# akanazawa/human_dynamics

Measured on AMD Instinct MI355X. Metric: frames/sec/GPU (ResNet+temporal+SMPL, 224x224); SMPL verts max-abs-err, higher is better.
Workload: dtype f16x3

## Files before the change

human_dynamics_amd/_lib.py:

```python
from __future__ import annotations

import ctypes as C
import os

from . import devflags

HERE = os.path.dirname(os.path.abspath(__file__))
LIB_PATH = devflags.get("LIB_PATH") or os.path.join(HERE, "libhmmr_hip.so")

HMMR_F32, HMMR_BF16, HMMR_F16X3 = 0, 1, 2
FLAG_SATURATED = 1
FLAG_NAN = 2
ABI_VERSION = 19
RESNET_UNITS = 16
RESNET_PROF_SLOTS = 64
MAX_TEMPORAL_BLOCKS = 8
MAX_REGRESSORS = 8

_vp, _fp, _ip = C.c_void_p, C.c_void_p, C.c_void_p


class ConvDesc(C.Structure):
    _fields_ = [
        ("in_", _vp), ("w", _vp), ("scale", _fp), ("shift", _fp), ("res", _vp), ("out", _vp),
        ("out2", _vp), ("scale2", _fp), ("shift2", _fp),
        ("in_dtype", C.c_int), ("out_dtype", C.c_int),
        ("n_img", C.c_int), ("hin", C.c_int), ("win", C.c_int), ("cin", C.c_int),
        ("in_img_stride", C.c_int64), ("in_row_stride", C.c_int), ("in_px_stride", C.c_int),
        ("kh", C.c_int), ("kw", C.c_int), ("sy", C.c_int), ("sx", C.c_int), ("py", C.c_int), ("px", C.c_int),
        ("ho", C.c_int), ("wo", C.c_int), ("cout", C.c_int), ("ldo", C.c_int),
        ("ldr", C.c_int), ("res_strided", C.c_int), ("res_img_stride", C.c_int64),
        ("res_row_stride", C.c_int), ("res_px_stride", C.c_int),
        ("relu", C.c_int), ("tile", C.c_int),
        ("split_k", C.c_int), ("ws", _vp), ("ws_bytes", C.c_size_t),
        ("pro_scale", _fp), ("pro_shift", _fp),
        ("out_b", _vp), ("ldo_b", C.c_int), ("n_split", C.c_int), ("relu_b", C.c_int),
        ("in2", _vp), ("cin2", C.c_int), ("k_order", C.c_int),
        ("batch", C.c_int), ("batch_in_bytes", C.c_int64), ("batch_w_bytes", C.c_int64), ("batch_out_bytes", C.c_int64),
        ("batch_res_bytes", C.c_int64), ("batch_scale_bytes", C.c_int64), ("batch_shift_bytes", C.c_int64),
    ]


class TailDesc(C.Structure):
    _fields_ = [
        ("dtype", C.c_int), ("h2", _vp), ("m", C.c_int), ("c_mid", C.c_int), ("depth", C.c_int),
        ("w3", _vp), ("scale3", _fp), ("shift3", _fp),
        ("res", _vp), ("ldr", C.c_int), ("res_strided", C.c_int), ("res_img_stride", C.c_int64),
        ("res_row_stride", C.c_int), ("res_px_stride", C.c_int), ("ho", C.c_int), ("wo", C.c_int),
        ("out", _vp), ("pre_scale", _fp), ("pre_shift", _fp),
        ("w1", _vp), ("scale1", _fp), ("shift1", _fp), ("relu1", C.c_int), ("n2", C.c_int),
        ("out_h1", _vp),
        ("h1", _vp), ("hin", C.c_int), ("win", C.c_int), ("w2", _vp), ("scale2", _fp), ("shift2", _fp),
        ("xp", _vp), ("wsc", _vp), ("shift_sc", _fp),
        ("conv2_stride", C.c_int), ("out_pre", _vp),
        ("pair_stream", _vp), ("c_xp", C.c_int), ("unit_stream", _vp), ("trunk_keep_stride", C.c_int),
    ]


class Debug(C.Structure):
    _fields_ = [("stem_route", C.c_int), ("stem_no_conv1", C.c_int), ("gemm_probe", C.c_int), ("smpl_blend_mfma", C.c_int), ("ief_no_group", C.c_int), ("reserved", C.c_int * 2), ("keep_dead_rows", C.c_int),
                ("pair_min_pixels", C.c_int), ("pair_two_tile_min", C.c_int), ("pair_form", C.c_int)]


class LaunchCounts(C.Structure):
    _fields_ = [("unit_pair", C.c_ulonglong), ("b1_unit", C.c_ulonglong), ("tail_split", C.c_ulonglong), ("conv3x3_stream", C.c_ulonglong),
                ("conv1x1_stream", C.c_ulonglong)]


class StemCounts(C.Structure):
    _fields_ = [(k, C.c_ulonglong) for k in ("fused", "fused_conv1", "repack", "gemm", "pool")]


TILE_GENERIC, TILE_PATCH, TILE_STREAM_3X3, TILE_STREAM_1X1 = range(4)
CONV_TILE_MAX = 63


class ConvTileInfo(C.Structure):
    _fields_ = [(k, C.c_int) for k in ("tile", "family", "fm", "fn", "wgm", "wgn", "pixels", "channels", "row_blocks", "depth", "occupancy", "wmax",
                                       "split_only", "conv3_form", "cols", "tune_cols", "narrow", "rank", "candidate")] + [("text", C.c_char_p)]


class Layer(C.Structure):
    _fields_ = [("w", _vp), ("scale", _fp), ("shift", _fp), ("tile", C.c_int), ("k_order", C.c_int)]


class ResnetUnit(C.Structure):
    _fields_ = [("conv1", Layer), ("conv2", Layer), ("conv3", Layer), ("shortcut", Layer), ("c3sc", Layer), ("sc_c1", Layer),
                ("w3_frag", _vp), ("w1n_frag", _vp), ("pair_stream", _vp), ("conv1_frag", _vp), ("unit_stream", _vp), ("pre_scale", _fp), ("pre_shift", _fp),
                ("c_in", C.c_int), ("base", C.c_int), ("depth", C.c_int), ("stride", C.c_int),
                ("fuse_preact", C.c_int), ("fuse_tail", C.c_int)]


class ResnetWeights(C.Structure):
    _fields_ = [("dtype", C.c_int), ("stem", Layer),
                ("unit", ResnetUnit * RESNET_UNITS), ("post_scale", _fp), ("post_shift", _fp)]


SC_NONE, SC_LAUNCH, SC_LAUNCH_WITH_CONV1, SC_IN_CONV3, SC_IN_TAIL = range(5)
CONV1_LAUNCH, CONV1_READY = range(2)
CONV2_LAUNCH, CONV2_IN_TAIL = range(2)
END_CONV3_LAUNCH, END_TAIL_BF16, END_TAIL_BF16_STRIDE2, END_TAIL_SPLIT, END_B1_UNIT, END_UNIT_PAIR = range(6)


class UnitPlan(C.Structure):
    _fields_ = [(k, C.c_int) for k in ("shortcut", "conv1", "conv2", "end", "reads_fused_preact", "writes_raw", "writes_pre",
                                       "pair_demoted", "swaps_t1_t2", "leaves_h1", "trunk_keep_stride")]


def resnet_plan(rw, n_total):
    plan = (UnitPlan * RESNET_UNITS)()
    check(load().hmmr_resnet50_plan(C.byref(rw), int(n_total), plan), "hmmr_resnet50_plan")
    return list(plan)

# ... 366 lines not shown
```

human_dynamics_amd/build.py:

```python
from __future__ import annotations

import os
import subprocess
import sys
from concurrent.futures import ThreadPoolExecutor

HERE = os.path.dirname(os.path.abspath(__file__))
CSRC = os.path.join(HERE, "csrc")
INCLUDE = os.path.join(os.path.dirname(HERE), "include")
LIB = os.path.join(HERE, "libhmmr_hip.so")
SOURCES = ["api.cpp", "pack.cpp", "gemm_conv.hip", "conv3x3_stream.hip", "conv1x1_stream.hip", "stem.hip", "bottleneck.hip", "bottleneck_split.hip", "unit_pair.hip", "b1_unit.hip", "resnet.hip", "temporal.hip", "ief.hip", "ief_grad.hip", "movie_grad.hip", "disc_pose.hip", "smpl.hip", "smpl_grad.hip", "losses.hip", "adam.hip", "eval_metrics.hip", "preprocess.hip", "tube.hip", "track.hip", "handoff.hip", "render.hip", "collage.hip", "person_view.hip", "windows.hip", "video_plan.cpp", "video.cpp", "probe.hip"]
HIPCC = os.environ.get("HIPCC", "/opt/rocm/bin/hipcc")
FLAGS = ["--offload-arch=gfx950", "-O3", "-std=c++17", "-fPIC", "-fno-slp-vectorize", "-I", INCLUDE, "-I", CSRC,
         "-Wall", "-Wno-unused-function"]


EXTRA_FLAGS = {"pack.cpp": ["-ffp-contract=off"], "track.hip": ["-ffp-contract=off"], "collage.hip": ["-ffp-contract=off"],
               "tube.hip": ["-ffp-contract=off"], "person_view.hip": ["-ffp-contract=off"], "adam.hip": ["-ffp-contract=off"]}


def _newer(src, dst):
    return (not os.path.exists(dst)) or os.path.getmtime(src) > os.path.getmtime(dst)


def _deps():
    return sorted(os.path.join(d, h) for d in (CSRC, INCLUDE) for h in os.listdir(d) if h.endswith(".h"))


def build(force=False, verbose=True):
    objs, jobs = [], []
    for src in SOURCES:
        s = os.path.join(CSRC, src)
        o = os.path.join(CSRC, os.path.splitext(src)[0] + ".o")
        objs.append(o)
        if force or _newer(s, o) or any(_newer(d, o) for d in _deps()):
            lang = ["-x", "hip"] if src.endswith(".hip") else []
            jobs.append([HIPCC] + FLAGS + EXTRA_FLAGS.get(src, []) + lang + ["-c", s, "-o", o])

    def run(cmd):
        if verbose:
            print(" ".join(cmd), flush=True)
        r = subprocess.run(cmd, stdout=subprocess.PIPE, stderr=subprocess.STDOUT, text=True)
        if r.returncode != 0:
            raise RuntimeError("hipcc failed:\n%s\n%s" % (" ".join(cmd), r.stdout))
        if verbose and r.stdout.strip():
            print(r.stdout)

    if jobs:
        with ThreadPoolExecutor(max_workers=min(len(jobs), os.cpu_count() or 4)) as ex:
            list(ex.map(run, jobs))
    if jobs or force or not os.path.exists(LIB):
        run([HIPCC, "--offload-arch=gfx950", "-shared", "-fPIC", "-o", LIB] + objs)
        from . import isa_check
        unsafe = isa_check.unsafe_forms(LIB)
        if unsafe:
            os.replace(LIB, LIB + ".rejected")
            raise RuntimeError("the linked library holds packed-fp32 instructions gfx950 gets wrong beside MFMAs (isa_check.py, DESIGN 4.6); "
                               "kept as %s.rejected:\n%s" % (LIB, "\n".join("  %d x %s %s in %s" % (n, op, mods, kern)
                                                                             for (kern, op, mods), n in sorted(unsafe.items()))))
        if verbose:
            print("isa_check: %s" % ("no disassembler (%s) or no gfx950 code object found in the library: NOT checked" % isa_check.OBJDUMP if unsafe is None
                                     else "no packed-fp32 instruction reads source 1's high register into its low result"), flush=True)
    return LIB

# ... 4 lines not shown
```

human_dynamics_amd/csrc/gemm_conv.hip:

```cpp
#include <stdlib.h>
#include <string.h>
#include <type_traits>

#include "conv_tiles.h"
#include "stream_kit.h"

struct ConvArgs {
    const void* in; const void* w; const float* scale; const float* shift;
    const void* res; void* out; void* out2; const float* scale2; const float* shift2;
    const float* pro_scale; const float* pro_shift;
    void* out_b; int ldo_b, n_split, relu_b;
    int M, K, cout, ldo, ldr;
    int Wo, HoWo, Hin, Win;
    long long in_img_stride; int in_row_stride, in_px_stride;
    int cin_log2, KH, KW, SY, SX, PY, PX;
    int res_strided; long long res_img_stride; int res_row_stride, res_px_stride;
    int relu, tiles_n, n_tiles;
    int kt_per_slice;
    long long out_slice_stride;
    int probe;
    const void* in2; int cin2, kt_split;
    int batch; long long bz_in, bz_w, bz_out, bz_res, bz_scale, bz_shift;
};

__device__ __forceinline__ ConvArgs batch_problem(const ConvArgs& a0, int z) {
    ConvArgs a = a0;
    if (a0.batch > 1) {
        const long long zz = z;
        a.in = (const char*)a0.in + zz * a0.bz_in;
        a.w = (const char*)a0.w + zz * a0.bz_w;
        if (a0.out) a.out = (char*)a0.out + zz * a0.bz_out;
        if (a0.out2) a.out2 = (char*)a0.out2 + zz * a0.bz_out;
        if (a0.res) a.res = (const char*)a0.res + zz * a0.bz_res;
        if (a0.scale) a.scale = (const float*)((const char*)a0.scale + zz * a0.bz_scale);
        if (a0.shift) a.shift = (const float*)((const char*)a0.shift + zz * a0.bz_shift);
        if (a0.scale2) a.scale2 = (const float*)((const char*)a0.scale2 + zz * a0.bz_scale);
        if (a0.shift2) a.shift2 = (const float*)((const char*)a0.shift2 + zz * a0.bz_shift);
    }
    return a;
}

#ifdef HMMR_GEMM_PROBE
#define HMMR_PROBE(a, bit) (((a).probe & (bit)) != 0)
#else
#define HMMR_PROBE(a, bit) false
#endif

template <typename TA> struct Frag;
template <> struct Frag<float>  { typedef f32x4 type; };
template <> struct Frag<bf16_t> { typedef bf16x8 type; };
struct split_frag { shalf8 hi, lo; };
template <> struct Frag<bsplit_t> { typedef split_frag type; };

__device__ __forceinline__ f32x16 mma(const f32x4& a, const f32x4& b, f32x16 c) {
#pragma unroll
    for (int j = 0; j < 4; ++j) c = __builtin_amdgcn_mfma_f32_32x32x2f32(a[j], b[j], c, 0, 0, 0);
    return c;
}
__device__ __forceinline__ f32x16 mma(const bf16x8& a, const bf16x8& b, f32x16 c) {
    return __builtin_amdgcn_mfma_f32_32x32x16_bf16(a, b, c, 0, 0, 0);
}
__device__ __forceinline__ f32x16 mma(const split_frag& a, const split_frag& b, f32x16 c) {
    c = mfma_split(a.lo, b.hi, c);
    c = mfma_split(a.hi, b.lo, c);
    return mfma_split(a.hi, b.hi, c);
}
template <typename TA> struct FragIO {
    static constexpr int CHUNKS = 4;
    __device__ static __forceinline__ typename Frag<TA>::type read(const char* row, int c, int lh, int fsw) {
        return *(const typename Frag<TA>::type*)(row + (((2 * c + lh) ^ fsw) << 4));
    }
};
template <> struct FragIO<bsplit_t> {
    static constexpr int CHUNKS = 2;
    __device__ static __forceinline__ split_frag read(const char* row, int c, int lh, int fsw) {
        const int g = 2 * (2 * c + lh);
        split_frag f;
        f.hi = *(const shalf8*)(row + ((g ^ fsw) << 4));
        f.lo = *(const shalf8*)(row + (((g + 1) ^ fsw) << 4));
        return f;
    }
};
template <typename TO> __device__ __forceinline__ void store_tail(TO* p, const float (&v)[8], int cnt) {
    if constexpr (!std::is_same<TO, bsplit_t>::value)
        for (int j = 0; j < cnt; ++j) p[j] = elem_traits<TO>::from_f32(v[j]);
}

__device__ const u32x4 g_zero_page[4] = {};

template <typename TA> __device__ __forceinline__ u32x4 preact_slot(const u32x4& v, const f32x4* sc, const f32x4* sh);
template <> __device__ __forceinline__ u32x4 preact_slot<float>(const u32x4& v, const f32x4* sc, const f32x4* sh) {
    u32x4 o;
#pragma unroll
    for (int i = 0; i < 4; ++i) o[i] = __float_as_uint(fmaxf(fmaf(__uint_as_float(v[i]), sc[0][i], sh[0][i]), 0.f));
    return o;
}
template <> __device__ __forceinline__ u32x4 preact_slot<bf16_t>(const u32x4& v, const f32x4* sc, const f32x4* sh) {
    u32x4 o;
#pragma unroll
    for (int i = 0; i < 4; ++i) {
        const float lo = __uint_as_float(v[i] << 16), hi = __uint_as_float(v[i] & 0xffff0000u);
        const int e = 2 * i;
        const float a = fmaxf(fmaf(lo, sc[e >> 2][e & 3], sh[e >> 2][e & 3]), 0.f);
        const float b = fmaxf(fmaf(hi, sc[(e + 1) >> 2][(e + 1) & 3], sh[(e + 1) >> 2][(e + 1) & 3]), 0.f);
        typedef __attribute__((ext_vector_type(2))) __bf16 bf16x2;
        bf16x2 pk = {(bf16_t)a, (bf16_t)b};
        o[i] = __builtin_bit_cast(unsigned, pk);
    }
    return o;
}


template <typename TA, typename TO, int BM, int BN, int WGM, int WGN, bool PRO, bool UTAP, int NSTAGE>
__global__ __launch_bounds__(WGM * WGN * 64, NSTAGE >= 3 ? (WGM * WGN) / 4 : ((WGM * WGN == 8) ? 4 : 1))
void conv_gemm_kernel(const ConvArgs a0) {
    const ConvArgs a = batch_problem(a0, blockIdx.z);
    static_assert(NSTAGE >= 2 && NSTAGE <= 4, "2 stages (two workgroups per CU) or a 3/4-stage ring (one workgroup per CU)");
    static_assert(NSTAGE == 2 || WGM * WGN == 8, "the deep ring is written for 8-wave workgroups");
    static_assert(!PRO || UTAP, "the fused pre-activation needs one tap per K step");
// ... 1030 lines not shown
```

human_dynamics_amd/csrc/ief.hip:

```cpp
#include "common.h"
#include "hmmr_hip.h"
#include "tail_sched.h"
#include "workspace.h"

template <typename TO>
__global__ void cast_rows_kernel(const float* __restrict__ in, TO* __restrict__ out, long long n8) {
    const long long i = (long long)blockIdx.x * blockDim.x + threadIdx.x;
    if (i >= n8) return;
    float v[8];
    load8(in + i * 8, v);
    store8(out + i * 8, v);
}

__global__ void ief_init_theta_kernel(const float* __restrict__ src, int ld_src, int off, int nd,
                                      float* __restrict__ theta, float* __restrict__ theta_other, int m, long long th_stride) {
    const long long i = (long long)blockIdx.x * blockDim.x + threadIdx.x;
    if (i >= (long long)m * LDT) return;
    const int row = (int)(i / LDT), col = (int)(i % LDT);
    const long long z = (long long)blockIdx.y * th_stride;
    theta[z + i] = col < nd ? src[(long long)row * ld_src + off + col] : 0.f;
    theta_other[z + i] = 0.f;
}

__global__ void ief_finalize_kernel(const float* __restrict__ theta, const float* __restrict__ bsrc, int ld_b,
// ... 44 lines not shown
extern "C" int hmmr_ief_fwd_from(const hmmr_ief_weights_t* w, const float* strips, const float* omega_start, int m,
                                 float* omegas, void* ws, size_t ws_bytes, void* stream) {
    HMMR_REQUIRE(w && strips && omegas && ws, "hmmr_ief_fwd: null argument");
    HMMR_REQUIRE(m > 0, "hmmr_ief_fwd: m must be positive");
    HMMR_REQUIRE(w->num_regressors >= 1 && w->num_regressors <= HMMR_MAX_REGRESSORS, "hmmr_ief_fwd: bad num_regressors");
    HMMR_REQUIRE(w->reg[0].nd == 85, "hmmr_ief_fwd: regressor 0 must predict 85-D omega");
    const int nd_delta = w->no_optcam ? 75 : 72;
    for (int r = 0; r < w->num_regressors; ++r)
        HMMR_REQUIRE(w->reg[r].nd == (r == 0 ? 85 : nd_delta), "hmmr_ief_fwd: regressor %d has nd=%d (expected %d)", r,
                     w->reg[r].nd, r == 0 ? 85 : nd_delta);
    const IefBufs L = ief_layout(m, w->dtype, w->num_regressors - 1);
    HMMR_REQUIRE(ws_bytes >= L.total, "hmmr_ief_fwd: workspace too small");
    hipStream_t s = (hipStream_t)stream;
    char* base = (char*)ws;
    const void* xin = strips;
    if (w->dtype != HMMR_F32) {
        const long long n8 = (long long)m * 2048 / 8;
        if (w->dtype == HMMR_BF16)
            hipLaunchKernelGGL(cast_rows_kernel<bf16_t>, dim3((unsigned)((n8 + 255) / 256)), dim3(256), 0, s, strips,
                               (bf16_t*)(base + L.xin), n8);
        else
            hipLaunchKernelGGL(cast_rows_kernel<bsplit_t>, dim3((unsigned)((n8 + 255) / 256)), dim3(256), 0, s, strips,
                               (bsplit_t*)(base + L.xin), n8);
        HMMR_CHECK_HIP(hipGetLastError());
        xin = base + L.xin;
    }
    void* pre = base + L.pre; void* h1 = base + L.h1; void* h2 = base + L.h2;
    float* th[2] = {(float*)(base + L.th[0]), (float*)(base + L.th[1])};
    const unsigned gth = (unsigned)(((long long)m * LDT + 255) / 256);
    const unsigned gfin = (unsigned)(((long long)m * 85 + 255) / 256);
    const int nd_group = w->num_regressors - 1;
    struct Strides { long long w, scale, shift; };
    auto strides_of = [&](const hmmr_layer_t hmmr_ief_regressor_t::*lay, Strides& st) -> bool {
        st = Strides{0, 0, 0};
        for (int r = 2; r < w->num_regressors; ++r) {
            const hmmr_layer_t& a = w->reg[r - 1].*lay; const hmmr_layer_t& b = w->reg[r].*lay;
            const Strides cur = {(const char*)b.w - (const char*)a.w,
                                 a.scale ? (const char*)b.scale - (const char*)a.scale : 0,
                                 a.shift ? (const char*)b.shift - (const char*)a.shift : 0};
            if (!a.scale != !b.scale || !a.shift != !b.shift) return false;
            if (r > 2 && (cur.w != st.w || cur.scale != st.scale || cur.shift != st.shift)) return false;
            st = cur;
        }
        return ((st.w | st.scale | st.shift) & 15) == 0;
    };
    Strides s_phi, s_th, s_fc2, s_fc3;
    const bool grouped = nd_group >= 2 && !hmmr_debug_state()->ief_no_group &&
                         strides_of(&hmmr_ief_regressor_t::fc1_phi, s_phi) && strides_of(&hmmr_ief_regressor_t::fc1_theta, s_th) &&
                         strides_of(&hmmr_ief_regressor_t::fc2, s_fc2) && strides_of(&hmmr_ief_regressor_t::fc3, s_fc3);
    const float* start = omega_start ? omega_start : w->mean_theta;
    const int ld_start = omega_start ? 85 : 0;
    const float* dsrc = w->delta_from_start ? start : (const float*)omegas;
    const int ld_d = w->delta_from_start ? ld_start : 85;
    auto run = [&](int r, int nb, const Strides& z_phi, const Strides& z_th, const Strides& z_fc2, const Strides& z_fc3) -> int {
        const hmmr_ief_regressor_t& R = w->reg[r];
        const long long ths = (long long)(L.th_s / 4);
        auto group = [&](hmmr_conv_desc_t& d, const Strides& z, long long in_b, long long out_b, long long res_b) {
            if (nb < 2) return;
            d.batch = nb; d.batch_in_bytes = in_b; d.batch_w_bytes = z.w; d.batch_out_bytes = out_b; d.batch_res_bytes = res_b;
            d.batch_scale_bytes = z.scale; d.batch_shift_bytes = z.shift;
        };
        if (r == 0)
            hipLaunchKernelGGL(ief_init_theta_kernel, dim3(gth), dim3(256), 0, s, start, ld_start, 0, 85, th[0], th[1], m, ths);
        else
            hipLaunchKernelGGL(ief_init_theta_kernel, dim3(gth, nb), dim3(256), 0, s, dsrc, ld_d, w->no_optcam ? 0 : 3, nd_delta,
                               th[0], th[1], m, ths);
        HMMR_CHECK_HIP(hipGetLastError());
        hmmr_conv_desc_t d = fc_desc(xin, w->dtype, m, 2048, R.fc1_phi, pre, w->dtype, 1024, 1024, IEF_SPLIT_K, base + L.sk, L.skbytes);
        group(d, z_phi, 0, (long long)L.pre_s, 0);
        if (hmmr_conv_gemm(&d, s)) return -2;
        int cur = 0;
        for (int st = 0; st < w->num_stages; ++st) {
            d = fc_desc(th[cur], HMMR_F32, m, LDT, R.fc1_theta, h1, w->dtype, 1024, 1024);
            d.res = pre; d.ldr = 1024; d.relu = 1;
            group(d, z_th, (long long)L.th_s, (long long)L.pre_s, (long long)L.pre_s);
            if (hmmr_conv_gemm(&d, s)) return -2;
            d = fc_desc(h1, w->dtype, m, 1024, R.fc2, h2, w->dtype, 1024, 1024, IEF_SPLIT_K, base + L.sk, L.skbytes);
            d.relu = 1;
            group(d, z_fc2, (long long)L.pre_s, (long long)L.pre_s, 0);
            if (hmmr_conv_gemm(&d, s)) return -2;
            d = fc_desc(h2, w->dtype, m, 1024, R.fc3, th[cur ^ 1], HMMR_F32, R.nd, LDT, IEF_SPLIT_K, base + L.sk, L.skbytes);
            d.res = th[cur]; d.ldr = LDT;
            group(d, z_fc3, (long long)L.pre_s, (long long)L.th_s, (long long)L.th_s);
            if (hmmr_conv_gemm(&d, s)) return -2;
            cur ^= 1;
        }
        hipLaunchKernelGGL(ief_finalize_kernel, dim3(gfin, nb), dim3(256), 0, s, (const float*)th[cur],
                           dsrc, ld_d, r == 0 ? 0 : (w->no_optcam ? 2 : 1), omegas + (size_t)r * m * 85, m, ths);
        HMMR_CHECK_HIP(hipGetLastError());
        return 0;
    };
    const Strides none = {0, 0, 0};
    if (run(0, 1, none, none, none, none)) return -2;
    if (grouped) return run(1, nd_group, s_phi, s_th, s_fc2, s_fc3);
    for (int r = 1; r < w->num_regressors; ++r)
        if (run(r, 1, none, none, none, none)) return -2;
    return 0;
}
```

human_dynamics_amd/csrc/stream_kit.h:

```cpp
#pragma once
#include <type_traits>
#include <utility>

#include "common.h"
#include "hmmr_hip.h"

template <class K, class... Args>
static int launch_with_lds(K kern, DeviceOnce& once, dim3 grid, dim3 block, int lds_attr, int lds, hipStream_t stream, Args... args) {
    if (const unsigned long long bit = once.due()) {
        HMMR_CHECK_HIP(hipFuncSetAttribute((const void*)kern, hipFuncAttributeMaxDynamicSharedMemorySize, lds_attr));
        once.mark(bit);
    }
    hipLaunchKernelGGL(kern, grid, block, lds, stream, args...);
    HMMR_CHECK_HIP(hipGetLastError());
    return 0;
}
static inline unsigned long long* probe_stamp_buffer() {
    const hmmr_debug_t* d = hmmr_debug_state();
    return (unsigned long long*)(((unsigned long long)(unsigned)d->reserved[1] << 32) | (unsigned)d->reserved[0]);
}

struct xfrag { shalf8 hi, lo; };
template <int V> using ic = std::integral_constant<int, V>;
template <class F, int... I> __device__ __forceinline__ void static_for(F&& f, std::integer_sequence<int, I...>) { (f(ic<I>{}), ...); }

typedef const __attribute__((address_space(1))) void* gptr_t;
typedef __attribute__((address_space(3))) void* lptr_t;
__device__ __forceinline__ unsigned lds_addr(void* p) { return (unsigned)(unsigned long long)(lptr_t)p; }

constexpr unsigned waitcnt_imm(int vm, int lgkm) { return (vm & 15) | (7 << 4) | (lgkm << 8) | ((vm >> 4) << 14); }
static_assert(waitcnt_imm(63, 0) == (63 | (7 << 4) | (0 << 8) | (3 << 14)) && waitcnt_imm(63, 0) == 0xC07F, "lgkmcnt(0) alone: the literal five files spelled out");
static_assert(waitcnt_imm(0, 0) == 0x0070 && waitcnt_imm(63, 15) == 0xCF7F, "everything; nothing");
static_assert(waitcnt_imm(63, 5) == 0xC57F && waitcnt_imm(37, 0) == 0x8075 && waitcnt_imm(37, 15) == 0x8F75, "lgkmcnt(5) alone; vmcnt(37) lgkmcnt(0); vmcnt(37) alone");
template <int N> __device__ __forceinline__ void wait_vm_lgkm0() {
    static_assert(N >= 0 && N < 64, "vmcnt is a 6-bit counter");
    __builtin_amdgcn_s_waitcnt(waitcnt_imm(N, 0));
}
template <int N> __device__ __forceinline__ void wait_vm() {
    static_assert(N >= 0 && N < 64, "vmcnt is a 6-bit counter");
    __builtin_amdgcn_s_waitcnt(waitcnt_imm(N, 15));
}
template <int N> __device__ __forceinline__ void wait_lgkm() {
    static_assert(N >= 0 && N <= 15, "lgkmcnt is a 4-bit counter");
    __builtin_amdgcn_s_waitcnt(waitcnt_imm(63, N));
}

template <class T, int OFF> __device__ __forceinline__ T lds_rd128(unsigned addr) {
    static_assert(sizeof(T) == 16, "a ds_read_b128");
    T v; asm volatile("ds_read_b128 %0, %1 offset:%2" : "=v"(v) : "v"(addr), "n"(OFF)); return v;
}
template <int OFF> __device__ __forceinline__ unsigned long long lds_rd64(unsigned addr) {
    unsigned long long v; asm volatile("ds_read_b64 %0, %1 offset:%2" : "=v"(v) : "v"(addr), "n"(OFF)); return v;
}
template <int OFF> __device__ __forceinline__ void lds_wr64(unsigned addr, unsigned long long v) {
    asm volatile("ds_write_b64 %0, %1 offset:%2" : : "v"(addr), "v"(v), "n"(OFF) : "memory");
}

static __device__ u32x4 g_dump_page[64 + 32] __attribute__((unused));

#ifndef TRUNK_DEAD_SHARED_PAGE
#define TRUNK_DEAD_SHARED_PAGE 0
#endif
constexpr int TRUNK_DEAD_WGS = 1024;
static __device__ u32x4 g_dead_rows[TRUNK_DEAD_WGS * 4 * 8] __attribute__((unused));
static_assert(sizeof(u32x4) * TRUNK_DEAD_WGS * 4 * 8 <= 512 * 1024, "the dead-row region lives in L2");
#define TRUNK_DEAD_ROW(wave, dlane) (TRUNK_DEAD_SHARED_PAGE ? (bsplit_t*)g_dump_page + lane * 4 \
                                     : (bsplit_t*)g_dead_rows + (((int)blockIdx.x & (TRUNK_DEAD_WGS - 1)) * 4 + (wave)) * 32 + (dlane))
static inline int trunk_keep_of(const hmmr_tail_desc_t* d) {
    const int s = hmmr_debug_state()->keep_dead_rows ? 0 : d->trunk_keep_stride;
    if (s > 1) hmmr_count_launch(HMMR_COUNT_TRUNK_KEEP);
    return s;
}
__device__ __forceinline__ unsigned trunk_live_mask(int mbase, int lane, int H, int W, int s) {
    if (s <= 1) return ~0u;
    asm volatile("" : "+s"(H), "+s"(W), "+s"(s));
    const unsigned m = (unsigned)(mbase + (lane & 31)), rem = m % (unsigned)(H * W), y = rem / (unsigned)W, x = rem - y * (unsigned)W;
    return (unsigned)__ballot(y % (unsigned)s == 0 && x % (unsigned)s == 0);
// ... 14 lines not shown
```

human_dynamics_amd/csrc/tail_sched.h:

```cpp
#pragma once
#include "common.h"
#include "hmmr_hip.h"

static constexpr int TAIL_C = 2048;
static constexpr float GN_EPS = 1e-6f;
static constexpr int GN_GROUPS = 32;
static constexpr int TEMPORAL_SPLIT_K_MAX = 5;
static inline int temporal_split_k(int dtype) { return dtype == HMMR_F16X3 ? 5 : 4; }
static constexpr int HAL_SPLIT_K = 4;

__device__ __forceinline__ float block_sum_256(float v, float* red) {
#pragma unroll
    for (int o = 32; o > 0; o >>= 1) v += __shfl_xor(v, o);
    __syncthreads();
    if ((threadIdx.x & 63) == 0) red[threadIdx.x >> 6] = v;
    __syncthreads();
    return red[0] + red[1] + red[2] + red[3];
}

static inline hmmr_conv_desc_t temporal_conv_desc(const void* in, int in_dtype, const hmmr_layer_t& l, const float* res, float* out, int b, int t,
                                                  void* sk, size_t skbytes) {
    constexpr int C = TAIL_C;
    hmmr_conv_desc_t d = {};
    d.in = in; d.w = l.w; d.scale = l.scale; d.shift = l.shift; d.tile = l.tile;
    d.out = out; d.in_dtype = in_dtype; d.out_dtype = HMMR_F32;
    d.n_img = b; d.hin = t; d.win = 1; d.cin = C;
    d.in_img_stride = (int64_t)t * C; d.in_row_stride = C; d.in_px_stride = C;
    d.kh = 3; d.kw = 1; d.sy = d.sx = 1; d.py = 1; d.px = 0; d.ho = t; d.wo = 1; d.cout = C; d.ldo = C;
    d.split_k = temporal_split_k(in_dtype); d.ws = sk; d.ws_bytes = skbytes;
    if (res) { d.res = res; d.ldr = C; }
    return d;
}

static inline hmmr_conv_desc_t fc_desc(const void* in, int in_dtype, int m, int k, const hmmr_layer_t& l, void* out, int out_dtype, int cout,
                                       int ldo, int split_k = 0, void* sk = nullptr, size_t skbytes = 0) {
    hmmr_conv_desc_t d = {};
    d.in = in; d.w = l.w; d.scale = l.scale; d.shift = l.shift; d.out = out;
    d.in_dtype = in_dtype; d.out_dtype = out_dtype;
    d.n_img = m; d.hin = d.win = 1; d.cin = k;
    d.in_img_stride = k; d.in_row_stride = k; d.in_px_stride = k;
    d.kh = d.kw = 1; d.sy = d.sx = 1; d.ho = d.wo = 1; d.cout = cout; d.ldo = ldo;
    if (split_k) { d.split_k = split_k; d.ws = sk; d.ws_bytes = skbytes; }
    return d;
}
static inline hmmr_conv_desc_t hal_fc_desc(const void* in, int in_dtype, const hmmr_layer_t& l, void* out, int out_dtype, int m, int relu,
                                           const float* res, void* sk, size_t skbytes) {
    hmmr_conv_desc_t d = fc_desc(in, in_dtype, m, TAIL_C, l, out, out_dtype, TAIL_C, TAIL_C, HAL_SPLIT_K, sk, skbytes);
    d.relu = relu; d.res = res; d.ldr = TAIL_C;
    return d;
}

static constexpr int LDT = 128;
static constexpr int IEF_SPLIT_K = 4;

__global__ void ief_finalize_kernel(const float* __restrict__ theta, const float* __restrict__ bsrc, int ld_b, int mode,
                                    float* __restrict__ out, int m, long long th_stride);
```

human_dynamics_amd/engine.py:

```python
from __future__ import annotations

import ctypes as C
import os
import threading
import time

import numpy as np
import torch

from . import _lib as L
from . import assets, devflags, packing

DTYPES = {"f32": L.HMMR_F32, "fp32": L.HMMR_F32, "float32": L.HMMR_F32,
          "bf16": L.HMMR_BF16, "bfloat16": L.HMMR_BF16,
          "f16x3": L.HMMR_F16X3, "split": L.HMMR_F16X3}
DTYPE_NAMES = {L.HMMR_F32: "f32", L.HMMR_BF16: "bf16", L.HMMR_F16X3: "f16x3"}
DEFAULT_DTYPE = "f16x3"
TILE_TABLES = os.path.join(os.path.dirname(os.path.abspath(__file__)), "tile_tables.json")


def set_debug(stem_route=0, stem_no_conv1=0, gemm_probe=0, smpl_blend_mfma=0, ief_no_group=0, pair_min_pixels=0, pair_two_tile_min=0, pair_form=0, keep_dead_rows=0):
    d = L.Debug()
    d.stem_route, d.stem_no_conv1, d.gemm_probe = int(stem_route), int(stem_no_conv1), int(gemm_probe)
    d.smpl_blend_mfma, d.ief_no_group, d.pair_min_pixels = int(smpl_blend_mfma), int(ief_no_group), int(pair_min_pixels)
    d.pair_two_tile_min, d.pair_form, d.keep_dead_rows = int(pair_two_tile_min), int(pair_form), int(keep_dead_rows)
    L.load().hmmr_set_debug(C.byref(d))


def _debug_from_env():
    e = devflags.get("STEM")
    c1 = devflags.get("STEM_C1")
    probe = int(devflags.get("GEMM_PROBE") or 0)
    if e or c1 == "0" or probe or _debug_from_env.was_set:
        set_debug(stem_route={"u": 1, "f": 2}.get(e[:1], 0), stem_no_conv1=int(c1 == "0"), gemm_probe=probe)
        _debug_from_env.was_set = bool(e or c1 == "0" or probe)


_debug_from_env.was_set = False


def _dt(d):
    if isinstance(d, str):
        if d == "bf16x3":
            import warnings
            warnings.warn("dtype 'bf16x3' is now 'f16x3' (split operands with fp16 halves since round 3)", DeprecationWarning, stacklevel=3)
            d = "f16x3"
        if d not in DTYPES:
            raise ValueError("unknown operand mode %r: use one of %s" % (d, ", ".join(sorted(set(DTYPES)))))
        return DTYPES[d]
    return int(d)


def _packer_choices(fold_sc=None, fuse_tail=None, patch_3x3=None, unit_pair=None, b1_stream=None, b1_unit=None, stem_conv1=True,
                    stream_1x1=None):
    def _flag_choice(name):
        v = devflags.get(name)
        return {"0": False, "1": True}.get(v, v)

    def pick(arg, flag):
        return flag if arg is None else arg
    fsc, fold = _flag_choice("FUSE_SC"), _flag_choice("FOLD_SC")
    return dict(fuse_preact_blocks=tuple(b for b in devflags.get("FUSE_PREACT").split(",") if b),
                fuse_tail=pick(fuse_tail, _flag_choice("FUSE_TAIL")),
                fuse_sc=fsc if isinstance(fsc, bool) else "all",
                fuse_preact_first=_flag_choice("PREACT_FIRST") is not False,
                fold_sc=pick(fold_sc, fold if isinstance(fold, bool) else None),
                patch_3x3=pick(patch_3x3, int(devflags.get("PATCH_3X3"))),
                unit_pair=pick(unit_pair, _flag_choice("UNIT_PAIR")),
                b1_stream=pick(b1_stream, _flag_choice("B1_STREAM") is True),
                b1_unit=pick(b1_unit, _flag_choice("B1_UNIT") is True),
                stem_conv1=stem_conv1,
                stream_1x1=pick(stream_1x1, _flag_choice("STREAM_1X1") is True))


class _Workspace(object):
# ... 1252 lines not shown
```

include/hmmr_hip.h:

```cpp
#ifndef HMMR_HIP_H
#define HMMR_HIP_H

#include <stddef.h>
#include <stdint.h>

#ifdef __cplusplus
extern "C" {
#endif

#define HMMR_ABI_VERSION 19

enum { HMMR_F32 = 0, HMMR_BF16 = 1, HMMR_F16X3 = 2 };

int hmmr_abi_version(void);
const char* hmmr_last_error(void);

#define HMMR_FLAG_SATURATED 1u
#define HMMR_FLAG_NAN 2u
int hmmr_run_flags(unsigned* flags, int clear);

typedef struct hmmr_debug_s {
    int stem_route;
    int stem_no_conv1;
    int gemm_probe;
    int smpl_blend_mfma;
    int ief_no_group;
    int reserved[2];
    int keep_dead_rows;
    int pair_min_pixels;
    int pair_two_tile_min;
    int pair_form;
} hmmr_debug_t;
void hmmr_set_debug(const hmmr_debug_t* d);
void hmmr_get_debug(hmmr_debug_t* d);

typedef struct {
    unsigned long long unit_pair;
    unsigned long long b1_unit;
    unsigned long long tail_split;
    unsigned long long conv3x3_stream;
    unsigned long long conv1x1_stream;
} hmmr_launch_counts_t;
void hmmr_launch_counts(hmmr_launch_counts_t* out, int clear);
unsigned long long hmmr_trunk_keep_launches(int clear);
typedef struct {
    unsigned long long fused;
    unsigned long long fused_conv1;
    unsigned long long repack;
    unsigned long long gemm;
    unsigned long long pool;
} hmmr_stem_counts_t;
void hmmr_stem_launch_counts(hmmr_stem_counts_t* out, int clear);

typedef struct {
    const void* in;
    const void* w;
    const float* scale;
    const float* shift;
    const void* res;
    void* out;
    void* out2;
    const float* scale2;
    const float* shift2;
    int in_dtype;
    int out_dtype;
    int n_img, hin, win, cin;
    int64_t in_img_stride;
    int in_row_stride, in_px_stride;
    int kh, kw, sy, sx, py, px;
    int ho, wo;
    int cout;
    int ldo;
    int ldr;
    int res_strided;
    int64_t res_img_stride;
    int res_row_stride, res_px_stride;
    int relu;
    int tile;
    int split_k;
    void* ws;
// ... 628 lines not shown
```

Baseline: 39680.

## Fuse IEF iterative regressor stages into one row-tiled persistent kernel

Adds an ief_rows kernel that, for f16x3, runs theta init, the fc1_theta/fc2/fc3 layers for every IEF stage and the finalize step inside one workgroup per 32-row tile. Hidden activations stay in LDS as split-half fragments instead of round-tripping through global memory across many GEMM launches. This is meant to remove per-stage launch overhead and intermediate traffic. In exchange it uses one 256-thread workgroup per CU with large LDS, which can limit parallelism when there are few rows. The debug reserved slot is repurposed as ief_form to select the old path, and the probe stamp pointer now reads from the renamed fields.

```diff
diff --git a/human_dynamics_amd/_lib.py b/human_dynamics_amd/_lib.py
--- a/human_dynamics_amd/_lib.py
+++ b/human_dynamics_amd/_lib.py
@@ -58,7 +58,7 @@
 
 
 class Debug(C.Structure):
-    _fields_ = [("stem_route", C.c_int), ("stem_no_conv1", C.c_int), ("gemm_probe", C.c_int), ("smpl_blend_mfma", C.c_int), ("ief_no_group", C.c_int), ("reserved", C.c_int * 2), ("keep_dead_rows", C.c_int),
+    _fields_ = [("stem_route", C.c_int), ("stem_no_conv1", C.c_int), ("gemm_probe", C.c_int), ("smpl_blend_mfma", C.c_int), ("ief_no_group", C.c_int), ("ief_form", C.c_int), ("reserved", C.c_int * 1), ("keep_dead_rows", C.c_int),
                 ("pair_min_pixels", C.c_int), ("pair_two_tile_min", C.c_int), ("pair_form", C.c_int)]
 
 
diff --git a/human_dynamics_amd/build.py b/human_dynamics_amd/build.py
--- a/human_dynamics_amd/build.py
+++ b/human_dynamics_amd/build.py
@@ -9,7 +9,7 @@
 CSRC = os.path.join(HERE, "csrc")
 INCLUDE = os.path.join(os.path.dirname(HERE), "include")
 LIB = os.path.join(HERE, "libhmmr_hip.so")
-SOURCES = ["api.cpp", "pack.cpp", "gemm_conv.hip", "conv3x3_stream.hip", "conv1x1_stream.hip", "stem.hip", "bottleneck.hip", "bottleneck_split.hip", "unit_pair.hip", "b1_unit.hip", "resnet.hip", "temporal.hip", "ief.hip", "ief_grad.hip", "movie_grad.hip", "disc_pose.hip", "smpl.hip", "smpl_grad.hip", "losses.hip", "adam.hip", "eval_metrics.hip", "preprocess.hip", "tube.hip", "track.hip", "handoff.hip", "render.hip", "collage.hip", "person_view.hip", "windows.hip", "video_plan.cpp", "video.cpp", "probe.hip"]
+SOURCES = ["api.cpp", "pack.cpp", "gemm_conv.hip", "conv3x3_stream.hip", "conv1x1_stream.hip", "stem.hip", "bottleneck.hip", "bottleneck_split.hip", "unit_pair.hip", "b1_unit.hip", "resnet.hip", "temporal.hip", "ief.hip", "ief_rows.hip", "ief_grad.hip", "movie_grad.hip", "disc_pose.hip", "smpl.hip", "smpl_grad.hip", "losses.hip", "adam.hip", "eval_metrics.hip", "preprocess.hip", "tube.hip", "track.hip", "handoff.hip", "render.hip", "collage.hip", "person_view.hip", "windows.hip", "video_plan.cpp", "video.cpp", "probe.hip"]
 HIPCC = os.environ.get("HIPCC", "/opt/rocm/bin/hipcc")
 FLAGS = ["--offload-arch=gfx950", "-O3", "-std=c++17", "-fPIC", "-fno-slp-vectorize", "-I", INCLUDE, "-I", CSRC,
          "-Wall", "-Wno-unused-function"]
diff --git a/human_dynamics_amd/csrc/gemm_conv.hip b/human_dynamics_amd/csrc/gemm_conv.hip
--- a/human_dynamics_amd/csrc/gemm_conv.hip
+++ b/human_dynamics_amd/csrc/gemm_conv.hip
@@ -49,22 +49,8 @@
 template <typename TA> struct Frag;
 template <> struct Frag<float>  { typedef f32x4 type; };
 template <> struct Frag<bf16_t> { typedef bf16x8 type; };
-struct split_frag { shalf8 hi, lo; };
 template <> struct Frag<bsplit_t> { typedef split_frag type; };
 
-__device__ __forceinline__ f32x16 mma(const f32x4& a, const f32x4& b, f32x16 c) {
-#pragma unroll
-    for (int j = 0; j < 4; ++j) c = __builtin_amdgcn_mfma_f32_32x32x2f32(a[j], b[j], c, 0, 0, 0);
-    return c;
-}
-__device__ __forceinline__ f32x16 mma(const bf16x8& a, const bf16x8& b, f32x16 c) {
-    return __builtin_amdgcn_mfma_f32_32x32x16_bf16(a, b, c, 0, 0, 0);
-}
-__device__ __forceinline__ f32x16 mma(const split_frag& a, const split_frag& b, f32x16 c) {
-    c = mfma_split(a.lo, b.hi, c);
-    c = mfma_split(a.hi, b.lo, c);
-    return mfma_split(a.hi, b.hi, c);
-}
 template <typename TA> struct FragIO {
     static constexpr int CHUNKS = 4;
     __device__ static __forceinline__ typename Frag<TA>::type read(const char* row, int c, int lh, int fsw) {
diff --git a/human_dynamics_amd/csrc/ief.hip b/human_dynamics_amd/csrc/ief.hip
--- a/human_dynamics_amd/csrc/ief.hip
+++ b/human_dynamics_amd/csrc/ief.hip
@@ -120,6 +120,7 @@
     const int ld_start = omega_start ? 85 : 0;
     const float* dsrc = w->delta_from_start ? start : (const float*)omegas;
     const int ld_d = w->delta_from_start ? ld_start : 85;
+    const bool fused = w->dtype == HMMR_F16X3 && hmmr_debug_state()->ief_form != 1;
     auto run = [&](int r, int nb, const Strides& z_phi, const Strides& z_th, const Strides& z_fc2, const Strides& z_fc3) -> int {
         const hmmr_ief_regressor_t& R = w->reg[r];
         const long long ths = (long long)(L.th_s / 4);
@@ -128,15 +129,33 @@
             d.batch = nb; d.batch_in_bytes = in_b; d.batch_w_bytes = z.w; d.batch_out_bytes = out_b; d.batch_res_bytes = res_b;
             d.batch_scale_bytes = z.scale; d.batch_shift_bytes = z.shift;
         };
-        if (r == 0)
-            hipLaunchKernelGGL(ief_init_theta_kernel, dim3(gth), dim3(256), 0, s, start, ld_start, 0, 85, th[0], th[1], m, ths);
-        else
-            hipLaunchKernelGGL(ief_init_theta_kernel, dim3(gth, nb), dim3(256), 0, s, dsrc, ld_d, w->no_optcam ? 0 : 3, nd_delta,
-                               th[0], th[1], m, ths);
-        HMMR_CHECK_HIP(hipGetLastError());
+        if (!fused) {
+            if (r == 0)
+                hipLaunchKernelGGL(ief_init_theta_kernel, dim3(gth), dim3(256), 0, s, start, ld_start, 0, 85, th[0], th[1], m, ths);
+            else
+                hipLaunchKernelGGL(ief_init_theta_kernel, dim3(gth, nb), dim3(256), 0, s, dsrc, ld_d, w->no_optcam ? 0 : 3, nd_delta,
+                                   th[0], th[1], m, ths);
+            HMMR_CHECK_HIP(hipGetLastError());
+        }
         hmmr_conv_desc_t d = fc_desc(xin, w->dtype, m, 2048, R.fc1_phi, pre, w->dtype, 1024, 1024, IEF_SPLIT_K, base + L.sk, L.skbytes);
         group(d, z_phi, 0, (long long)L.pre_s, 0);
         if (hmmr_conv_gemm(&d, s)) return -2;
+        const int fin_mode = r == 0 ? 0 : (w->no_optcam ? 2 : 1);
+        if (fused) {
+            ief_rows_args_t q = {};
+            if (r == 0) { q.src = start; q.ld_src = ld_start; q.off = 0; q.nd = 85; }
+            else { q.src = dsrc; q.ld_src = ld_d; q.off = w->no_optcam ? 0 : 3; q.nd = nd_delta; }
+            q.pre = (const bsplit_t*)pre; q.th[0] = th[0]; q.th[1] = th[1];
+            const hmmr_layer_t* lay[3] = {&R.fc1_theta, &R.fc2, &R.fc3};
+            const Strides* zs[3] = {&z_th, &z_fc2, &z_fc3};
+            for (int l = 0; l < 3; ++l) {
+                q.w[l] = lay[l]->w; q.scale[l] = lay[l]->scale; q.shift[l] = lay[l]->shift;
+                q.z_w[l] = zs[l]->w; q.z_scale[l] = zs[l]->scale; q.z_shift[l] = zs[l]->shift;
+            }
+            q.bsrc = dsrc; q.ld_b = ld_d; q.mode = fin_mode; q.out = omegas + (size_t)r * m * 85;
+            q.m = m; q.stages = w->num_stages; q.z_pre = (long long)L.pre_s; q.z_th = ths;
+            return ief_rows_launch(q, nb, s) ? -2 : 0;
+        }
         int cur = 0;
         for (int st = 0; st < w->num_stages; ++st) {
             d = fc_desc(th[cur], HMMR_F32, m, LDT, R.fc1_theta, h1, w->dtype, 1024, 1024);
@@ -154,7 +173,7 @@
             cur ^= 1;
         }
         hipLaunchKernelGGL(ief_finalize_kernel, dim3(gfin, nb), dim3(256), 0, s, (const float*)th[cur],
-                           dsrc, ld_d, r == 0 ? 0 : (w->no_optcam ? 2 : 1), omegas + (size_t)r * m * 85, m, ths);
+                           dsrc, ld_d, fin_mode, omegas + (size_t)r * m * 85, m, ths);
         HMMR_CHECK_HIP(hipGetLastError());
         return 0;
     };
diff --git a/human_dynamics_amd/csrc/ief_rows.hip b/human_dynamics_amd/csrc/ief_rows.hip
--- /dev/null
+++ b/human_dynamics_amd/csrc/ief_rows.hip
@@ -0,0 +1,343 @@
+#include "stream_kit.h"
+#include "tail_sched.h"
+
+namespace {
+constexpr int RT = 32;
+constexpr int HID = 1024;
+constexpr int H_ROW = HID * 4;
+constexpr int OFF_TH = RT * H_ROW;
+constexpr int OFF_SC = OFF_TH + RT * LDT * 4;
+constexpr int LDS_BYTES = OFF_SC + 4 * 32 * 32 * 4;
+static_assert(LDS_BYTES <= 160 * 1024, "one workgroup per CU: 160 KB of LDS");
+constexpr int NK = HID / 32;
+constexpr int SL0 = IEF_SPLIT_K > NK ? NK : (IEF_SPLIT_K > 1 ? IEF_SPLIT_K : 1);
+constexpr int KPS = (NK + SL0 - 1) / SL0;
+constexpr int NSL = (NK + KPS - 1) / KPS;
+constexpr int NF3 = 3;
+static_assert(NSL * RT * NF3 * 32 * 4 <= OFF_TH, "fc3's partial planes reuse the split tile");
+static_assert(LDT == 128 && LDT % 32 == 0, "theta rows are whole 128-byte K steps");
+
+typedef const __attribute__((address_space(1))) char* grow_t;
+typedef const __attribute__((address_space(1))) shalf8* gsh8_t;
+typedef const __attribute__((address_space(1))) f32x4* gf4_t;
+
+__device__ __forceinline__ int h_off(int row, int slot) { return row * H_ROW + ((slot ^ (row & 15)) << 4); }
+__device__ __forceinline__ int th_idx(int row, int col) { return row * LDT + ((((col >> 2) ^ (row & 15)) << 2) | (col & 3)); }
+
+template <int N> __device__ __forceinline__ void zero(f32x16 (&acc)[N]) {
+#pragma unroll
+    for (int j = 0; j < N; ++j)
+#pragma unroll
+        for (int r = 0; r < 16; ++r) acc[j][r] = 0.f;
+}
+__device__ __forceinline__ void scale_shift(float (&v)[8], const float* scale, const float* shift, int n) {
+    if (scale && shift) {
+        float s[8], b[8]; load8(scale + n, s); load8(shift + n, b);
+#pragma unroll
+        for (int j = 0; j < 8; ++j) v[j] = fmaf(v[j], s[j], b[j]);
+    } else if (scale) {
+        float s[8]; load8(scale + n, s);
+#pragma unroll
+        for (int j = 0; j < 8; ++j) v[j] *= s[j];
+    } else if (shift) {
+        float b[8]; load8(shift + n, b);
+#pragma unroll
+        for (int j = 0; j < 8; ++j) v[j] += b[j];
+    }
+}
+__device__ __forceinline__ void frag_to_scratch(float* ssc, const f32x16& acc, int lr, int lh) {
+#pragma unroll
+    for (int r = 0; r < 16; ++r) ssc[((r & 3) + 8 * (r >> 2) + 4 * lh) * 32 + lr] = acc[r];
+}
+}
+
+__global__ __launch_bounds__(256, 1) void ief_rows_kernel(const ief_rows_args_t a0) {
+    extern __shared__ __attribute__((aligned(16))) char smem[];
+    const long long z = blockIdx.y;
+    const ief_rows_args_t& a = a0;
+    const bsplit_t* pre = (const bsplit_t*)((const char*)a0.pre + z * a0.z_pre);
+    float* th0 = a0.th[0] + z * a0.z_th;
+    float* th1 = a0.th[1] + z * a0.z_th;
+    float* out = a0.out + z * a0.m * 85;
+    const char* w1 = (const char*)a0.w[0] + z * a0.z_w[0];
+    const char* w2 = (const char*)a0.w[1] + z * a0.z_w[1];
+    const char* w3 = (const char*)a0.w[2] + z * a0.z_w[2];
+#define IEF_ROWS_VEC(name, field, l) const float* name = a0.field[l] ? (const float*)((const char*)a0.field[l] + z * a0.z_##field[l]) : nullptr
+    IEF_ROWS_VEC(sc1, scale, 0); IEF_ROWS_VEC(sc2, scale, 1); IEF_ROWS_VEC(sc3, scale, 2);
+    IEF_ROWS_VEC(sh1, shift, 0); IEF_ROWS_VEC(sh2, shift, 1); IEF_ROWS_VEC(sh3, shift, 2);
+#undef IEF_ROWS_VEC
+    const int tid = threadIdx.x, lane = tid & 63;
+    const int wave = __builtin_amdgcn_readfirstlane(tid >> 6);
+    const int lr = lane & 31, lh = lane >> 5, sw = lr & 15;
+    const int m0 = blockIdx.x * RT, M = a.m;
+    float* sth = (float*)(smem + OFF_TH);
+    float* ssc = (float*)(smem + OFF_SC) + wave * 1024;
+    float satmax = 0.f;
+    const char* ah[2][2][2];
+    const char* at[2][4];
+#pragma unroll
+    for (int k1 = 0; k1 < 2; ++k1) {
+#pragma unroll
+        for (int c = 0; c < 2; ++c)
+#pragma unroll
+            for (int p = 0; p < 2; ++p) ah[k1][c][p] = smem + lr * H_ROW + ((((8 * k1 + 4 * c + p) | (2 * lh)) ^ sw) << 4);
+#pragma unroll
+        for (int c = 0; c < 4; ++c) at[k1][c] = smem + OFF_TH + lr * LDT * 4 + ((((8 * k1 + 2 * c) | lh) ^ sw) << 4);
+    }
+    static_assert(KPS % 2 == 0 || NSL == 1, "fc3 starts a slice on an even K step");
+
+    for (int i = tid; i < RT * LDT; i += 256) {
+        const int row = i / LDT, col = i % LDT, m = m0 + row;
+        float v = 0.f;
+        if (m < M) {
+            if (col < a.nd) v = a.src[(long long)m * a.ld_src + a.off + col];
+            th0[(long long)m * LDT + col] = v;
+            th1[(long long)m * LDT + col] = 0.f;
+        }
+        sth[th_idx(row, col)] = v;
+    }
+    __syncthreads();
+
+    int cur = 0;
+    for (int st = 0; st < a.stages; ++st, cur ^= 1) {
+        asm volatile("" ::: "memory");
+#pragma unroll 1
+        for (int half = 0; half < 2; ++half) {
+            const int n0 = wave * 256 + half * 128;
+            grow_t wj[4];
+#pragma unroll
+            for (int j = 0; j < 4; ++j) { wj[j] = (grow_t)(w1 + (long long)(n0 + j * 32 + lr) * (LDT * 4) + lh * 16); asm volatile("" : "+v"(wj[j])); }
+            f32x16 acc[4];
+            zero(acc);
+            f32x4 fb[2][4][4];
+            auto fetch = [&](int kt, int buf) {
+#pragma unroll
+                for (int c = 0; c < 4; ++c)
+#pragma unroll
+                    for (int j = 0; j < 4; ++j) fb[buf][c][j] = *(gf4_t)(wj[j] + (kt * 8 + 2 * c) * 16);
+            };
+            fetch(0, 0);
+#pragma unroll
+            for (int kt = 0; kt < LDT / 32; ++kt) {
+                if (kt + 1 < LDT / 32) fetch(kt + 1, (kt + 1) & 1);
+                __builtin_amdgcn_sched_barrier(0);
+#pragma unroll
+                for (int c = 0; c < 4; ++c) {
+                    const f32x4 fa = *(const f32x4*)(at[kt & 1][c] + 256 * (kt >> 1));
+#pragma unroll
+                    for (int j = 0; j < 4; ++j) acc[j] = mma(fa, fb[kt & 1][c][j], acc[j]);
+                }
+                __builtin_amdgcn_sched_barrier(0);
+            }
+#pragma unroll
+            for (int j = 0; j < 4; ++j) {
+                frag_to_scratch(ssc, acc[j], lr, lh);
+                __syncthreads();
+#pragma unroll
+                for (int it = 0; it < 2; ++it) {
+                    const int idx = it * 64 + lane, row = idx >> 2, col = (idx & 3) * 8;
+                    const int m = m0 + row, n = n0 + j * 32 + col;
+                    float v[8];
+                    load8(ssc + row * 32 + col, v);
+                    scale_shift(v, sc1, sh1, n);
+                    if (m < M) {
+                        const u32x4* rp = (const u32x4*)(pre + (long long)m * HID + n);
+                        const u32x4 rres[2] = {rp[0], rp[1]};
+                        float rr[8];
+                        unpack8<bsplit_t>(rres, rr);
+#pragma unroll
+                        for (int q = 0; q < 8; ++q) v[q] += rr[q];
+                    }
+#pragma unroll
+                    for (int q = 0; q < 8; ++q) v[q] = fmaxf(v[q], 0.f);
+                    if (m < M) satmax = sat_acc(sat_acc(sat_acc(sat_acc(satmax, v[0], v[1]), v[2], v[3]), v[4], v[5]), v[6], v[7]);
+                    unsigned h[4], l[4];
+#pragma unroll
+                    for (int q = 0; q < 4; ++q) split2_mix(split_clamp(v[2 * q]), split_clamp(v[2 * q + 1]), h[q], l[q]);
+                    *(u32x4*)(smem + h_off(row, n >> 2)) = u32x4{h[0], h[1], h[2], h[3]};
+                    *(u32x4*)(smem + h_off(row, (n >> 2) + 1)) = u32x4{l[0], l[1], l[2], l[3]};
+                }
+                __syncthreads();
+            }
+        }
+
+        f32x16 sum[4][2];
+#pragma unroll
+        for (int q = 0; q < 4; ++q) {
+            const int n0 = wave * 256 + q * 64;
+            grow_t wj[2];
+#pragma unroll
+            for (int j = 0; j < 2; ++j) { wj[j] = (grow_t)(w2 + (long long)(n0 + j * 32 + lr) * H_ROW + lh * 32); asm volatile("" : "+v"(wj[j])); }
+            split_frag fb[4][2][2];
+            auto fetch = [&](int kt, int buf) {
+#pragma unroll
+                for (int j = 0; j < 2; ++j)
+#pragma unroll
+                    for (int c = 0; c < 2; ++c) {
+                        const gsh8_t p = (gsh8_t)(wj[j] + (kt * 4 + 2 * c) * 32);
+                        fb[buf][j][c].hi = p[0]; fb[buf][j][c].lo = p[1];
+                    }
+            };
+            f32x16 acc[2];
+            zero(acc);
+#pragma unroll
+            for (int kt = 0; kt < 3 && kt < NK; ++kt) fetch(kt, kt);
+#pragma unroll
+            for (int kt = 0; kt < NK; ++kt) {
+                if (kt + 3 < NK) fetch(kt + 3, (kt + 3) % 4);
+                __builtin_amdgcn_sched_barrier(0);
+                split_frag fa[2];
+#pragma unroll
+                for (int c = 0; c < 2; ++c) {
+                    fa[c].hi = *(const shalf8*)(ah[kt & 1][c][0] + 256 * (kt >> 1));
+                    fa[c].lo = *(const shalf8*)(ah[kt & 1][c][1] + 256 * (kt >> 1));
+                }
+#pragma unroll
+                for (int c = 0; c < 2; ++c)
+#pragma unroll
+                    for (int j = 0; j < 2; ++j) acc[j] = mma(fa[c], fb[kt % 4][j][c], acc[j]);
+                if (kt % KPS == KPS - 1 || kt == NK - 1) {
+#pragma unroll
+                    for (int j = 0; j < 2; ++j) {
+                        if (kt < KPS) sum[q][j] = acc[j];
+                        else sum[q][j] += acc[j];
+                    }
+                    zero(acc);
+                }
+                __builtin_amdgcn_sched_barrier(0);
+            }
+        }
+        __syncthreads();
+#pragma unroll
+        for (int q = 0; q < 4; ++q)
+#pragma unroll
+            for (int j = 0; j < 2; ++j) {
+                const int n0 = wave * 256 + q * 64;
+                frag_to_scratch(ssc, sum[q][j], lr, lh);
+                __syncthreads();
+#pragma unroll
+                for (int it = 0; it < 2; ++it) {
+                    const int idx = it * 64 + lane, row = idx >> 2, col = (idx & 3) * 8;
+                    const int m = m0 + row, n = n0 + j * 32 + col;
+                    float v[8];
+                    load8(ssc + row * 32 + col, v);
+                    scale_shift(v, sc2, sh2, n);
+#pragma unroll
+                    for (int e = 0; e < 8; ++e) v[e] = fmaxf(v[e], 0.f);
+                    if (m < M) satmax = sat_acc(sat_acc(sat_acc(sat_acc(satmax, v[0], v[1]), v[2], v[3]), v[4], v[5]), v[6], v[7]);
+                    shalf8 hi, lo;
+#pragma unroll
+                    for (int e = 0; e < 8; ++e) {
+                        const float c = split_clamp(v[e]);
+                        hi[e] = (shalf_t)c;
+                        lo[e] = (shalf_t)(c - (float)hi[e]);
+                    }
+                    *(shalf8*)(smem + h_off(row, n >> 2)) = hi;
+                    *(shalf8*)(smem + h_off(row, (n >> 2) + 1)) = lo;
+                }
+                __syncthreads();
+            }
+
+        f32x16 acc3[(NSL + 3) / 4][NF3];
+#pragma unroll
+        for (int si = 0; si < (NSL + 3) / 4; ++si) {
+            zero(acc3[si]);
+            const int sl = si * 4 + wave;
+            if (sl < NSL) {
+                const int kt0 = sl * KPS;
+                grow_t wj[NF3];
+#pragma unroll
+                for (int j = 0; j < NF3; ++j) { wj[j] = (grow_t)(w3 + (long long)(j * 32 + lr) * H_ROW + lh * 32 + (long long)kt0 * 128); asm volatile("" : "+v"(wj[j])); }
+                split_frag fb[3][NF3][2];
+                auto fetch = [&](int kt, int buf) {
+#pragma unroll
+                    for (int j = 0; j < NF3; ++j)
+#pragma unroll
+                        for (int c = 0; c < 2; ++c) {
+                            const gsh8_t p = (gsh8_t)(wj[j] + (kt * 4 + 2 * c) * 32);
+                            fb[buf][j][c].hi = p[0]; fb[buf][j][c].lo = p[1];
+                        }
+                };
+                const int n = min(KPS, NK - kt0);
+                fetch(0, 0);
+                if (1 < n) fetch(1, 1);
+#pragma unroll
+                for (int i = 0; i < KPS; ++i) {
+                    if (i < n) {
+                        if (i + 2 < n) fetch(i + 2, (i + 2) % 3);
+                        __builtin_amdgcn_sched_barrier(0);
+                        split_frag fa[2];
+#pragma unroll
+                        for (int c = 0; c < 2; ++c) {
+                            fa[c].hi = *(const shalf8*)(ah[i & 1][c][0] + 256 * (kt0 >> 1) + 256 * (i >> 1));
+                            fa[c].lo = *(const shalf8*)(ah[i & 1][c][1] + 256 * (kt0 >> 1) + 256 * (i >> 1));
+                        }
+#pragma unroll
+                        for (int c = 0; c < 2; ++c)
+#pragma unroll
+                            for (int j = 0; j < NF3; ++j) acc3[si][j] = mma(fa[c], fb[i % 3][j][c], acc3[si][j]);
+                    }
+                }
+            }
+        }
+        __syncthreads();
+        float* planes = (float*)smem;
+#pragma unroll
+        for (int si = 0; si < (NSL + 3) / 4; ++si) {
+            const int sl = si * 4 + wave;
+            if (sl < NSL)
+#pragma unroll
+                for (int j = 0; j < NF3; ++j)
+#pragma unroll
+                    for (int r = 0; r < 16; ++r)
+                        planes[(sl * RT + (r & 3) + 8 * (r >> 2) + 4 * lh) * (NF3 * 32) + j * 32 + lr] = acc3[si][j][r];
+        }
+        __syncthreads();
+        {
+            const int vpr = (a.nd + 7) / 8;
+            float* tho = cur ? th0 : th1;
+            for (int i = tid; i < RT * vpr; i += 256) {
+                const int row = i / vpr, n = (i % vpr) * 8, m = m0 + row;
+                float v[8];
+                load8(planes + row * (NF3 * 32) + n, v);
+                for (int s = 1; s < NSL; ++s) {
+                    float p[8];
+                    load8(planes + (s * RT + row) * (NF3 * 32) + n, p);
+#pragma unroll
+                    for (int q = 0; q < 8; ++q) v[q] += p[q];
+                }
+                scale_shift(v, sc3, sh3, n);
+                const int cnt = min(8, a.nd - n);
+#pragma unroll
+                for (int q = 0; q < 8; ++q) {
+                    if (q < cnt) {
+                        const float t = v[q] + sth[th_idx(row, n + q)];
+                        sth[th_idx(row, n + q)] = t;
+                        if (m < M) tho[(long long)m * LDT + n + q] = t;
+                    }
+                }
+            }
+        }
+        __syncthreads();
+    }
+    split_flag_max(satmax);
+
+    for (int i = tid; i < RT * 85; i += 256) {
+        const int row = i / 85, col = i % 85, m = m0 + row;
+        if (m >= M) continue;
+        float v;
+        if (a.mode == 0) v = sth[th_idx(row, col)];
+        else if (col >= 75) v = a.bsrc[(long long)m * a.ld_b + col];
+        else if (a.mode == 2) v = sth[th_idx(row, col)];
+        else if (col == 0) v = 1.f;
+        else if (col < 3) v = 0.f;
+        else v = sth[th_idx(row, col - 3)];
+        out[(long long)m * 85 + col] = v;
+    }
+}
+
+int ief_rows_launch(const ief_rows_args_t& a, int nb, hipStream_t stream) {
+    static DeviceOnce once;
+    return launch_with_lds(ief_rows_kernel, once, dim3((unsigned)((a.m + RT - 1) / RT), (unsigned)nb), dim3(256), LDS_BYTES, LDS_BYTES,
+                           stream, a);
+}
diff --git a/human_dynamics_amd/csrc/stream_kit.h b/human_dynamics_amd/csrc/stream_kit.h
--- a/human_dynamics_amd/csrc/stream_kit.h
+++ b/human_dynamics_amd/csrc/stream_kit.h
@@ -17,12 +17,27 @@
 }
 static inline unsigned long long* probe_stamp_buffer() {
     const hmmr_debug_t* d = hmmr_debug_state();
-    return (unsigned long long*)(((unsigned long long)(unsigned)d->reserved[1] << 32) | (unsigned)d->reserved[0]);
+    return (unsigned long long*)(((unsigned long long)(unsigned)d->reserved[0] << 32) | (unsigned)d->ief_form);
 }
 
 struct xfrag { shalf8 hi, lo; };
 template <int V> using ic = std::integral_constant<int, V>;
 template <class F, int... I> __device__ __forceinline__ void static_for(F&& f, std::integer_sequence<int, I...>) { (f(ic<I>{}), ...); }
+
+struct split_frag { shalf8 hi, lo; };
+__device__ __forceinline__ f32x16 mma(const f32x4& a, const f32x4& b, f32x16 c) {
+#pragma unroll
+    for (int j = 0; j < 4; ++j) c = __builtin_amdgcn_mfma_f32_32x32x2f32(a[j], b[j], c, 0, 0, 0);
+    return c;
+}
+__device__ __forceinline__ f32x16 mma(const bf16x8& a, const bf16x8& b, f32x16 c) {
+    return __builtin_amdgcn_mfma_f32_32x32x16_bf16(a, b, c, 0, 0, 0);
+}
+__device__ __forceinline__ f32x16 mma(const split_frag& a, const split_frag& b, f32x16 c) {
+    c = mfma_split(a.lo, b.hi, c);
+    c = mfma_split(a.hi, b.lo, c);
+    return mfma_split(a.hi, b.hi, c);
+}
 
 typedef const __attribute__((address_space(1))) void* gptr_t;
 typedef __attribute__((address_space(3))) void* lptr_t;
diff --git a/human_dynamics_amd/csrc/tail_sched.h b/human_dynamics_amd/csrc/tail_sched.h
--- a/human_dynamics_amd/csrc/tail_sched.h
+++ b/human_dynamics_amd/csrc/tail_sched.h
@@ -53,5 +53,17 @@
 static constexpr int LDT = 128;
 static constexpr int IEF_SPLIT_K = 4;
 
+struct ief_rows_args_t {
+    const float* src; int ld_src, off, nd;
+    const bsplit_t* pre;
+    const void* w[3]; const float* scale[3]; const float* shift[3];
+    float* th[2];
+    const float* bsrc; int ld_b, mode;
+    float* out;
+    int m, stages;
+    long long z_pre, z_th, z_w[3], z_scale[3], z_shift[3];
+};
+int ief_rows_launch(const ief_rows_args_t& a, int nb, hipStream_t stream);
+
 __global__ void ief_finalize_kernel(const float* __restrict__ theta, const float* __restrict__ bsrc, int ld_b, int mode,
                                     float* __restrict__ out, int m, long long th_stride);
diff --git a/human_dynamics_amd/engine.py b/human_dynamics_amd/engine.py
--- a/human_dynamics_amd/engine.py
+++ b/human_dynamics_amd/engine.py
@@ -19,8 +19,9 @@
 TILE_TABLES = os.path.join(os.path.dirname(os.path.abspath(__file__)), "tile_tables.json")
 
 
-def set_debug(stem_route=0, stem_no_conv1=0, gemm_probe=0, smpl_blend_mfma=0, ief_no_group=0, pair_min_pixels=0, pair_two_tile_min=0, pair_form=0, keep_dead_rows=0):
+def set_debug(stem_route=0, stem_no_conv1=0, gemm_probe=0, smpl_blend_mfma=0, ief_no_group=0, pair_min_pixels=0, pair_two_tile_min=0, pair_form=0, keep_dead_rows=0, ief_form=0):
     d = L.Debug()
+    d.ief_form = int(ief_form)
     d.stem_route, d.stem_no_conv1, d.gemm_probe = int(stem_route), int(stem_no_conv1), int(gemm_probe)
     d.smpl_blend_mfma, d.ief_no_group, d.pair_min_pixels = int(smpl_blend_mfma), int(ief_no_group), int(pair_min_pixels)
     d.pair_two_tile_min, d.pair_form, d.keep_dead_rows = int(pair_two_tile_min), int(pair_form), int(keep_dead_rows)
diff --git a/include/hmmr_hip.h b/include/hmmr_hip.h
--- a/include/hmmr_hip.h
+++ b/include/hmmr_hip.h
@@ -25,7 +25,8 @@
     int gemm_probe;
     int smpl_blend_mfma;
     int ief_no_group;
-    int reserved[2];
+    int ief_form;
+    int reserved[1];
     int keep_dead_rows;
     int pair_min_pixels;
     int pair_two_tile_min;
```

Measured after the change: 39320. No clear change (-0.9%).
